# meyer-lab/cmtf-pls

Hardware: AMD Instinct MI355X
Metric: nipals_iters_per_sec (higher is better)
Workload: dtype f32

## Files before the change

cmtf_pls_amd/_lib.py:

```python
from __future__ import annotations

import ctypes
import os
from ctypes import c_char_p, c_double, c_int, c_int64, c_size_t, c_uint32, c_uint64, c_void_p

_HERE = os.path.dirname(os.path.abspath(__file__))
LIB_PATH = os.environ.get("CMTFPLS_LIB") or os.path.join(_HERE, "lib", "libcmtfpls.so")

_P = c_void_p

class XcovBlock(ctypes.Structure):
    _fields_ = [("S", _P), ("S2", _P), ("colcnt", _P), ("n_samples", c_double), ("order", c_int), ("A", c_int), ("B", c_int),
                ("n_squarings", c_int), ("Z", _P), ("wA", _P), ("wB", _P), ("info", _P)]


class KfoldState(ctypes.Structure):
    _fields_ = [("I", c_int), ("A", c_int), ("B", c_int), ("M", c_int), ("K", c_int), ("R", c_int)] + [
        (name, _P) for name in ("fold_of", "S", "mean", "Yk", "Gy", "WA", "WB", "Q", "Wa", "Wb", "T", "Gt", "coef", "Rm", "tm",
                                "Tout", "vec", "n_iter", "status", "part")]


class CvCoupledBlock(ctypes.Structure):
    _fields_ = [("X", _P), ("order", c_int), ("A", c_int), ("B", c_int)]

# ... 42 lines not shown
    "cmtfpls_project_rows2_idx_f64": (c_int, [_P, c_int, c_int, _P, _P, _P, _P, c_int, c_int, _P, _P, _P, _P, c_int64, c_int, _P, c_int, _P]),
    "cmtfpls_allreduce_sum_f64": (c_int, [_P, _P, c_size_t, _P]),
    "cmtfpls_allreduce_sum_f32": (c_int, [_P, _P, c_size_t, _P]),
    "cmtfpls_axpy_scalar_f64": (c_int, [_P, c_int64, _P, _P, _P]),
    "cmtfpls_xcov_deflate_f32": (c_int, [_P, c_int64, c_int, c_int, _P, c_int, c_int, _P, _P, _P, _P, _P, _P, c_size_t, _P]),
    "cmtfpls_xcov_deflate_f64": (c_int, [_P, c_int64, c_int, c_int, _P, c_int, c_int, _P, _P, _P, _P, _P, _P, c_size_t, _P]),
    "cmtfpls_xcov_stats_workspace_bytes": (c_size_t, [c_int64, c_int64, c_int]),
    "cmtfpls_xcov_stats_f32": (c_int, [_P, c_int64, c_int64, _P, c_int, c_int, _P, _P, _P, c_size_t, _P]),
    "cmtfpls_xcov_stats_f64": (c_int, [_P, c_int64, c_int64, _P, c_int, c_int, _P, _P, _P, c_size_t, _P]),
    "cmtfpls_xcov_ssq_workspace_bytes": (c_size_t, [c_int64, c_int64, c_int]),
    "cmtfpls_xcov_ssq_f32": (c_int, [_P, c_int64, c_int64, _P, c_int, c_int, _P, _P, _P, _P, c_size_t, _P]),
    "cmtfpls_xcov_ssq_f64": (c_int, [_P, c_int64, c_int64, _P, c_int, c_int, _P, _P, _P, _P, c_size_t, _P]),
    "cmtfpls_score_contract_workspace_bytes": (c_size_t, [c_int64, c_int64]),
    "cmtfpls_score_contract_f32": (c_int, [_P, c_int64, c_int, c_int, _P, _P, _P, _P, _P, c_double, _P, _P, _P, _P, c_size_t, _P]),
    "cmtfpls_score_contract_f64": (c_int, [_P, c_int64, c_int, c_int, _P, _P, _P, _P, _P, c_double, _P, _P, _P, _P, c_size_t, _P]),
    "cmtfpls_kr_axpy_f64": (c_int, [_P, c_int, c_int, _P, _P, c_int, c_int, _P, _P]),
    "cmtfpls_xcov_f32_mixed": (c_int, [_P, c_int64, c_int64, _P, c_int, c_int, _P, c_int, _P, c_size_t, _P]),
    "cmtfpls_mttkrp_f32_mixed": (c_int, [_P, c_int64, c_int, c_int, _P, _P, c_int, _P, c_int, _P]),
    "cmtfpls_mttkrp_f32": (c_int, [_P, c_int64, c_int, c_int, _P, _P, c_int, _P, c_int, _P]),
    "cmtfpls_mttkrp_f64": (c_int, [_P, c_int64, c_int, c_int, _P, _P, c_int, _P, c_int, _P]),
    "cmtfpls_score_f32": (c_int, [_P, c_int64, c_int, c_int, _P, _P, _P, _P, _P]),
    "cmtfpls_score_f64": (c_int, [_P, c_int64, c_int, c_int, _P, _P, _P, _P, _P]),
    "cmtfpls_score_s_f64": (c_int, [_P, c_int, c_int, c_int, _P, _P, _P, _P]),
    "cmtfpls_deflate_contract_workspace_bytes": (c_size_t, [c_int64, c_int64]),
    "cmtfpls_deflate_contract_yq_f32": (c_int, [_P, c_int64, c_int, c_int, _P, _P, _P, _P, c_int, c_int, _P, _P, c_int, _P, _P, c_size_t, _P]),
    "cmtfpls_deflate_contract_yq_f64": (c_int, [_P, c_int64, c_int, c_int, _P, _P, _P, _P, c_int, c_int, _P, _P, c_int, _P, _P, c_size_t, _P]),
    "cmtfpls_score_gram_f32": (c_int, [_P, c_int64, c_int, c_int, _P, _P, _P, _P, _P, c_int, c_int, _P, _P]),
    "cmtfpls_score_gram_f64": (c_int, [_P, c_int64, c_int, c_int, _P, _P, _P, _P, _P, c_int, c_int, _P, _P]),
    "cmtfpls_q_update_f64": (c_int, [_P, c_int, c_int, _P, c_int, _P, _P, _P, _P]),
    "cmtfpls_deflate_f32": (c_int, [_P, c_int64, c_int, c_int, _P, _P, _P, _P, _P]),
# ... 128 lines not shown
```

cmtf_pls_amd/backend.py:

```python
from __future__ import annotations

import ctypes
from typing import Optional, Tuple

import torch

from . import _lib

_SUFFIX = {torch.float32: "f32", torch.float64: "f64"}


def _ptr(t: Optional[torch.Tensor]):
    return None if t is None else t.data_ptr()


def _int_pairs(pairs):
    flat = [int(v) for p in pairs for v in p]
    return (ctypes.c_int * len(flat))(*flat)


class HipBackend:
    name = "hip"

    def __init__(self, device: Optional[torch.device] = None):
# ... 297 lines not shown
        if rc == 4:
            return None
        _lib.check(rc, "mttkrp")
        return out

    def score(self, X2, A, B, wA, wB, rowcnt, out) -> torch.Tensor:
        _lib.check(self._fn("score", X2)(_ptr(X2), X2.shape[0], A, B, _ptr(wA), _ptr(wB), _ptr(rowcnt), _ptr(out), self._stream()), "score")
        return out

    def score_s(self, S, A, B, wA, wB, out) -> torch.Tensor:
        assert S.dtype == torch.float64 and S.is_contiguous()
        _lib.check(self.lib.cmtfpls_score_s_f64(_ptr(S), S.shape[0], A, B, _ptr(wA), _ptr(wB), _ptr(out), self._stream()), "score_s")
        return out

    def score_contract(self, X2, A, B, wA, wB, shift, t, Z, sub_own=None, add_other=None, alpha: float = 1.0,
                       csum: Optional[torch.Tensor] = None) -> Optional[torch.Tensor]:
        I, P = X2.shape
        if not X2.is_contiguous() or P != A * B:
            return None
        for v in (sub_own, add_other):
            assert v is None or (v.is_contiguous() and v.numel() == I and v.dtype == torch.float64)
        nbytes = self.lib.cmtfpls_score_contract_workspace_bytes(I, P)
        ws = self._workspace("score_contract", max(nbytes, 256))
        rc = self._fn("score_contract", X2)(_ptr(X2), I, A, B, _ptr(wA), _ptr(wB), _ptr(shift), _ptr(sub_own), _ptr(add_other), float(alpha),
                                            _ptr(t), _ptr(Z), _ptr(csum), _ptr(ws), ws.numel(), self._stream())
        if rc == 4:
            return None
        _lib.check(rc, "score_contract")
        return Z

    def score_gram(self, X2, A, B, wA, wB, rowcnt, out, Y: torch.Tensor, qpart: torch.Tensor) -> Optional[torch.Tensor]:
        assert qpart.numel() >= self.n_partials * Y.shape[1] and qpart.is_contiguous()
        rc = self._fn("score_gram", X2)(_ptr(X2), X2.shape[0], A, B, _ptr(wA), _ptr(wB), _ptr(rowcnt), _ptr(out),
                                        _ptr(Y), Y.stride(0), Y.shape[1], _ptr(qpart), self._stream())
        if rc == 4:
            return None
        _lib.check(rc, "score_gram")
        return out

    def q_update(self, q: torch.Tensor, qpart: Optional[torch.Tensor] = None, normalize: bool = True,
                 G: Optional[torch.Tensor] = None, q_prev: Optional[torch.Tensor] = None,
                 du2: Optional[torch.Tensor] = None, nparts: Optional[int] = None) -> None:
        M = q.numel()
# ... 619 lines not shown
```

cmtf_pls_amd/csrc/scorecontract.hip:

```cpp
#include "common.hpp"

namespace cmtfpls {

void launch_reduce_rows(const double* part, int nrows, int64_t P, double* out, hipStream_t st);

constexpr int kScGrid = 256;

template <int CTRL>
__device__ __forceinline__ double dpp_move(double v) {
  const uint64_t b = __double_as_longlong(v);
  const uint32_t lo = (uint32_t)__builtin_amdgcn_update_dpp(0, (int)(uint32_t)b, CTRL, 0xf, 0xf, false);
  const uint32_t hi = (uint32_t)__builtin_amdgcn_update_dpp(0, (int)(uint32_t)(b >> 32), CTRL, 0xf, 0xf, false);
  return __longlong_as_double(((uint64_t)hi << 32) | lo);
}
__device__ __forceinline__ double row16_sum(double v) {
  v += dpp_move<0xB1>(v);
  v += dpp_move<0x4E>(v);
  v += dpp_move<0x141>(v);
  v += dpp_move<0x140>(v);
  return v;
}

constexpr int kScLdsA = 2048;
template <typename T, int NV, bool KC, bool WL = false>
__global__ __launch_bounds__(1024) void score_contract_rows_kernel(const T* __restrict__ X, int64_t I, unsigned P, int B,
                                                                  const double* __restrict__ wA, const double* __restrict__ wB,
                                                                  const double* __restrict__ shift, const double* __restrict__ sub_own,
                                                                  const double* __restrict__ add_other, double alpha,
                                                                  double* __restrict__ t, double* __restrict__ part,
                                                                  double* __restrict__ csum_part) {
  __shared__ double red[2][16];
  __shared__ double wls[WL ? kScLdsA : 1];
  constexpr int V = VecOf<T>::N;
  using VT = Pack<T, V>;
  constexpr unsigned stride = 1024u * V;
  const unsigned c0 = threadIdx.x * V;
  const int lane = threadIdx.x & 63, wv = threadIdx.x >> 6;
  double wa[WL ? 1 : NV], wb[KC ? 1 : NV][V], acc[NV][V];
  bool ok[NV];
  const unsigned j0 = c0 / (unsigned)B, jstep = stride / (unsigned)B;
  if constexpr (WL) {
    for (unsigned j = threadIdx.x; j < NV * jstep; j += 1024) wls[(j % jstep) * NV + j / jstep] = wA[j];
    __syncthreads();
  }
#pragma unroll
// ... 7 lines not shown
      if (!KC || n == 0) wb[KC ? 0 : n][e] = wB[cg % (unsigned)B + e];
      acc[n][e] = 0.0;
    }
  }
  const double sh = shift ? shift[0] : 0.0;
  unsigned col[WL ? 1 : NV];
  if constexpr (!WL) {
#pragma unroll
    for (int n = 0; n < NV; ++n) col[n] = ok[n] ? c0 + n * stride : 0u;
  }
  const int64_t step = gridDim.x;
  int64_t r = blockIdx.x;
  VT bufA[NV], bufB[NV];
  int parity = 0;
  double csum = 0.0;
  auto load = [&](VT (&buf)[NV], int64_t row) {
#pragma unroll
    for (int n = 0; n < NV; ++n) {
      if constexpr (WL) {
        const uint64_t o = (uint64_t)(row * (int64_t)P + (int64_t)n * stride);
        const uint64_t ou = ((uint64_t)__builtin_amdgcn_readfirstlane((uint32_t)(o >> 32)) << 32) | __builtin_amdgcn_readfirstlane((uint32_t)o);
        buf[n] = ld_stream(reinterpret_cast<const VT*>(X + ou + c0));
      } else {
        buf[n] = ld_stream(reinterpret_cast<const VT*>(X + row * (int64_t)P + col[n]));
      }
    }
  };
  auto use = [&](VT (&buf)[NV], int64_t row) {
    double d = 0.0;
#pragma unroll
    for (int n = 0; n < NV; ++n) {
      double dn = 0.0;
#pragma unroll
      for (int e = 0; e < V; ++e) dn = fma((double)buf[n].e[e], wb[KC ? 0 : n][e], dn);
      d = fma(WL ? wls[j0 * NV + n] : wa[WL ? 0 : n], dn, d);
    }
    d = wave_sum(d);
    if (lane == 0) red[parity][wv] = d;
    __syncthreads();
    double ti = row16_sum(red[parity][lane & 15]) - sh;
    parity ^= 1;
    if (sub_own) ti -= sub_own[row];
    if (threadIdx.x == 0) t[row] = ti;
    if (add_other) ti += add_other[row];
    ti *= alpha;
    csum += ti;
    if constexpr (sizeof(T) == 4) {
#pragma unroll
      for (int n = 0; n < NV; ++n)
#pragma unroll
        for (int e = 0; e < V; ++e) asm volatile("" : "+v"(buf[n].e[e]));
    }
#pragma unroll
    for (int n = 0; n < NV; ++n)
#pragma unroll
      for (int e = 0; e < V; ++e) acc[n][e] = fma(ti, (double)buf[n].e[e], acc[n][e]);
  };
  const int64_t last = I - 1;
  if (r < I) load(bufA, r);
  while (r < I) {
    const int64_t r1 = r + step;
    load(bufB, r1 < I ? r1 : last);
    use(bufA, r);
    if (r1 >= I) break;
    const int64_t r2 = r1 + step;
    load(bufA, r2 < I ? r2 : last);
    use(bufB, r1);
    r = r2;
  }
  if (csum_part && threadIdx.x == 0) csum_part[blockIdx.x] = csum;
  double* __restrict__ prow = part + (int64_t)blockIdx.x * P + c0;
#pragma unroll
  for (int n = 0; n < NV; ++n)
    if (ok[n]) {
#pragma unroll
      for (int e = 0; e < V; ++e) prow[n * stride + e] = acc[n][e];
    }
}

constexpr unsigned long long kXchEmpty = ~0ull;
constexpr int kSplitMaxG = 16;
constexpr int kSplitSpinLimit = 1 << 21;

__global__ __launch_bounds__(256) void xch_preset_kernel(unsigned long long* __restrict__ p, int64_t n) {
  for (int64_t i = (int64_t)blockIdx.x * 256 + threadIdx.x; i < n; i += (int64_t)gridDim.x * 256) p[i] = kXchEmpty;
// ... 125 lines not shown
}

static int split_cus() {
  static int cus = 0;
  if (cus == 0) {
    int dev = 0, n = 0;
    if (hipGetDevice(&dev) != hipSuccess || hipDeviceGetAttribute(&n, hipDeviceAttributeMultiprocessorCount, dev) != hipSuccess || n <= 0) n = 256;
    cus = n;
  }
  return cus;
}

template <typename T>
static int run_score_contract(const T* X, int64_t I, int A, int B, const double* wA, const double* wB, const double* shift,
                              const double* sub_own, const double* add_other, double alpha, double* t, double* Z, double* csum,
                              void* ws, size_t ws_bytes, hipStream_t st) {
  if (!X || !wA || !wB || !t || !Z || I <= 0 || A <= 0 || B <= 0) { set_error("score_contract: bad argument"); return CMTFPLS_EINVAL; }
  constexpr int V = 16 / (int)sizeof(T);
  const int64_t P = (int64_t)A * B;
  const int64_t stride = (int64_t)1024 * V;
  const int nv = (int)((P + stride - 1) / stride);
  constexpr int kMaxNV = (V == 4) ? 4 : 8;
  if ((B % V) != 0 || P < stride / 2 || P >= ((int64_t)1 << 31) || (reinterpret_cast<uintptr_t>(X) & 15) != 0) {
    set_error("score_contract: shape outside the row-in-registers form; use score + mode0_contract");
    return CMTFPLS_EUNSUPPORTED;
  }
  const bool kc = (stride % B) == 0;
  if (nv > kMaxNV) {
    const int NVS = (sizeof(T) == 4 && !kc) ? 2 : 4;
    const int G = (nv + NVS - 1) / NVS;
    const int cus = split_cus() < kScGrid ? split_cus() : kScGrid;
    const int S = (int)(I < cus / G ? I : cus / G);
    if (G > kSplitMaxG || S < 1) {
      set_error("score_contract: row beyond 16 workgroups' registers; use score + mode0_contract");
      return CMTFPLS_EUNSUPPORTED;
    }
    const size_t need = ((size_t)S * (P + 1) + (size_t)I * G) * sizeof(double);
    if (!ws || ws_bytes < need) { set_error("score_contract: workspace too small"); return CMTFPLS_EWORKSPACE; }
    double* part = static_cast<double*>(ws);
    double* csum_part = part + (size_t)S * P;
    unsigned long long* xch = reinterpret_cast<unsigned long long*>(csum_part + S);
    hipLaunchKernelGGL(xch_preset_kernel, dim3((unsigned)(((int64_t)I * G + 2047) / 2048)), dim3(256), 0, st, xch, (int64_t)I * G);
// ... 1 lines not shown
  hipLaunchKernelGGL((score_contract_split_kernel<T, NVV, KCC, LG>), dim3(S * G), dim3(1024), 0, st, X, I, (unsigned)P, B, G, wA, wB, \
                     shift, sub_own, add_other, alpha, t, part, csum ? csum_part : nullptr, xch)
    if constexpr (sizeof(T) == 8) {
      if (kc) SPL(4, true, 2);
      else SPL(4, false, 1);
    } else {
      if (kc) SPL(4, true, 1);
      else SPL(2, false, 2);
    }
#undef SPL
    launch_reduce_rows(part, S, P, Z, st);
    if (csum) launch_reduce_rows(csum_part, S, 1, csum, st);
    return check_launch("score_contract (split rows)");
  }
  const int grid = (int)(I < kScGrid ? I : kScGrid);
  if (!ws || ws_bytes < (size_t)grid * (P + 1) * sizeof(double)) { set_error("score_contract: workspace too small"); return CMTFPLS_EWORKSPACE; }
  double* part = static_cast<double*>(ws);
  double* csum_part = csum ? part + (size_t)grid * P : nullptr;
#define SCL(NVV)                                                                                                                  \
  do {                                                                                                                            \
    if (kc) hipLaunchKernelGGL((score_contract_rows_kernel<T, NVV, true>), dim3(grid), dim3(1024), 0, st, X, I, (unsigned)P, B, wA, wB, shift, sub_own, add_other, alpha, t, part, csum_part); \
    else hipLaunchKernelGGL((score_contract_rows_kernel<T, NVV, false>), dim3(grid), dim3(1024), 0, st, X, I, (unsigned)P, B, wA, wB, shift, sub_own, add_other, alpha, t, part, csum_part); \
  } while (0)
  if (nv <= 1) SCL(1);
  else if (nv <= 2) SCL(2);
  else if (nv <= 4) SCL(4);
  else if constexpr (kMaxNV >= 8) {
    if (kc && P == 8 * stride && A <= kScLdsA)
      hipLaunchKernelGGL((score_contract_rows_kernel<T, 8, true, true>), dim3(grid), dim3(1024), 0, st, X, I, (unsigned)P, B, wA, wB, shift, sub_own, add_other, alpha, t, part, csum_part);
    else SCL(8);
  }
#undef SCL
  launch_reduce_rows(part, grid, P, Z, st);
  if (csum) launch_reduce_rows(csum_part, grid, 1, csum, st);
  return check_launch("score_contract");
}

}

using namespace cmtfpls;

extern "C" {
size_t cmtfpls_score_contract_workspace_bytes(int64_t I, int64_t P) {
  if (I <= 0 || P <= 0) return 0;
  return ((size_t)(I < kScGrid ? I : kScGrid) * (size_t)(P + 1) + (size_t)I * kSplitMaxG) * sizeof(double);
}
int cmtfpls_score_contract_f32(const float* X, int64_t I, int A, int B, const double* wA, const double* wB, const double* shift,
                               const double* sub_own, const double* add_other, double alpha, double* t, double* Z, double* csum,
                               void* ws, size_t ws_bytes, void* stream) {
  return run_score_contract<float>(X, I, A, B, wA, wB, shift, sub_own, add_other, alpha, t, Z, csum, ws, ws_bytes, (hipStream_t)stream);
}
int cmtfpls_score_contract_f64(const double* X, int64_t I, int A, int B, const double* wA, const double* wB, const double* shift,
                               const double* sub_own, const double* add_other, double alpha, double* t, double* Z, double* csum,
                               void* ws, size_t ws_bytes, void* stream) {
  return run_score_contract<double>(X, I, A, B, wA, wB, shift, sub_own, add_other, alpha, t, Z, csum, ws, ws_bytes, (hipStream_t)stream);
}
}
```

cmtf_pls_amd/csrc/small.hip:

```cpp
#include "common.hpp"

namespace cmtfpls {

void launch_reduce_rows(const double* part, int nrows, int64_t P, double* out, hipStream_t st);

constexpr int kSmallBlocks = 128;
constexpr int kMaxGramDim = 64;
constexpr size_t kSmallWsBytes = (size_t)kSmallBlocks * kMaxGramDim * kMaxGramDim * sizeof(double);

__global__ __launch_bounds__(256) void gram_tn_kernel(const double* __restrict__ A, int lda, int a,
                                                     const double* __restrict__ B, int ldb, int b,
                                                     int64_t I, double* __restrict__ part, int TR) {
  extern __shared__ double lds[];
  double* As = lds;
  double* Bs = lds + TR * a;
  const int ab = a * b;
  const int64_t rows_per = (I + gridDim.x - 1) / gridDim.x;
  const int64_t r0 = (int64_t)blockIdx.x * rows_per;
  const int64_t r1 = (r0 + rows_per < I) ? r0 + rows_per : I;
  double acc[16];
#pragma unroll
  for (int s = 0; s < 16; ++s) acc[s] = 0.0;
  for (int64_t rb = r0; rb < r1; rb += TR) {
    const int nr = (int)((r1 - rb < TR) ? r1 - rb : TR);
// ... 207 lines not shown
    if (lane < M) {
      q[lane] = v;
      if (G) dq[lane] = v - q_prev[lane];
    }
  }
  if (G) {
    __syncthreads();
    double sacc = 0.0;
    for (int idx = tid; idx < M * M; idx += 1024) {
      const int i = idx / M, j = idx - i * M;
      sacc = fma(dq[i] * G[idx], dq[j], sacc);
    }
    sacc = block_sum(sacc, red);
    if (tid == 0) du2[0] = sacc;
  }
}

__global__ __launch_bounds__(256) void s_downdate_kernel(double* __restrict__ S, int M, int64_t P, int B,
                                                        const double* __restrict__ ya, const double* __restrict__ wA,
                                                        const double* __restrict__ wB, const double* __restrict__ q,
                                                        const double* __restrict__ v) {
  const int64_t c = (int64_t)blockIdx.x * 256 + threadIdx.x;
  if (c >= P) return;
  const double w = wA[c / B] * wB[c % B];
  const double vc = v[c];
  for (int m = 0; m < M; ++m) {
    double sv = S[(int64_t)m * P + c];
    sv = fma(-ya[m], w, sv);
    sv = fma(-q[m], vc, sv);
    S[(int64_t)m * P + c] = sv;
// ... 224 lines not shown
```

cmtf_pls_amd/fitrun.py:

```python
from __future__ import annotations

import math
from typing import Dict, List, Optional

import numpy as np
import torch

from .fitrun_xcov import XcovMixin
from .state import BlockState, FitState, split_trailing, validate_limits


class FitRun(XcovMixin):

    def __init__(self, eng: NipalsEngine, Xs: List[torch.Tensor], Y: torch.Tensor, n_components: int, coupled: bool,
                 algorithm: str = "direct", owned: Optional[List[bool]] = None, allow_raw: bool = True):
        be, comm = eng.be, eng.comm
        Xs = list(Xs)
        owned = [True] * len(Xs) if owned is None else list(owned)
        if algorithm not in ("direct", "xcov"):
            raise ValueError("algorithm must be 'direct' or 'xcov'")
        self.algorithm_requested = self.algorithm = algorithm
        self.notes: List[str] = []
        validate_limits([tuple(X.shape) for X in Xs], n_components)
        self.eng, self.Xs, self.Y, self.R, self.coupled = eng, Xs, Y, n_components, coupled
# ... 136 lines not shown
                self.one.fill_(1.0)
                self.vs = [be.empty(blk.A * blk.B) for blk in self.blocks]
                self._nowrite = eng.opt.xcov_nowrite and hasattr(be, "kr_axpy") and R <= 64
                if self._nowrite:
                    self.dot_log = be.zeros(R, 1 + len(self.blocks))
                    self.Gw = be.empty(R * R)
                    self._G_last = None
                    self._one_read = R > 1 and eng.opt.xcov_one_read and hasattr(be, "score_contract")
                    if self._one_read:
                        self._fused_b = max(range(len(self.blocks)), key=lambda b: self.blocks[b].A * self.blocks[b].B)
                        P0 = self.blocks[self._fused_b].A * self.blocks[self._fused_b].B
                        self.ps = be.empty(P0)
                        self.Rm = be.zeros(P0, R)
                        self.corr = be.empty(I)
                        self.csum = be.empty(1)
            assert self._nowrite or not self.raw, "an uncentred X needs the form of the loop that never writes it"

    def _blocks_from_one_read(self, Xs: List[torch.Tensor]) -> Optional[List[BlockState]]:
        be, comm = self.eng.be, self.eng.comm
        blocks, n = [], float(self.n_total)
        for b, X in enumerate(Xs):
            I = X.shape[0]
            X2 = X.view(I, -1)
            P = X2.shape[1]
            out = be.xcov_stats(X2, self.Y, out=be.empty(self.M, P))
            if out is None:
                return None
            S, stats = out
            comm.allreduce(stats)
            colsum, colsq = stats[:P], stats[P:]
            ssq = (colsq - colsum * colsum / n).sum().reshape(1)
# ... 483 lines not shown
            rep["x_passes_per_component"] = ("1 read + write (deflation fused with the next contraction)" if self._fused
                                             else "1 read + write (deflation)")
            rep["x_copy"] = "centred private copy"
        else:
            nowrite = bool(getattr(self, "_nowrite", False))
            one_read = nowrite and bool(getattr(self, "_one_read", False))
            any_miss = any(b.has_miss for b in self.blocks)
            rep["x_copy"] = "none: the caller's uncentred tensor is read in place" if self.raw else "centred private copy"
            rep["raw"] = bool(self.raw)
            rep["x_written"] = not nowrite
            rep["s_carried"] = bool(self._s_carry)
            rep["s_build"] = ("per component (missing values)" if any_miss else "first component only") + \
                             (f", {(self.M + 63) // 64} response tiles of <= 64" if self.M > 64 else "") + \
                             (", [Y, Y * rowscale] in one pass" if any(x is not None for x in self.S12) else "")
            rep["one_read"] = one_read
            rep["stats_with_s"] = bool(getattr(self, "_stats_with_s", False))
            if nowrite:
                rep["x_passes_per_component"] = ("1 read (largest block); 2 reads (other blocks)" if one_read and nb > 1 else
                                                 "1 read" if one_read else "2 reads")
            elif any_miss and nb == 1 and getattr(self, "_deflate_build_ok", True) and self.S12[0] is not None and eng.opt.xcov_deflate_build:
                rep["x_passes_per_component"] = "1 read + 1 read + write (deflation inside the rebuild of S)"
            elif any_miss:
                rep["x_passes_per_component"] = "1 read + write (score + deflation) + S rebuild reads"
            else:
                rep["x_passes_per_component"] = "1 read + 1 read + write"
            rep["pipelined"] = bool(getattr(self, "_pipelined", False))
            if rep["pipelined"]:
                rep["pipeline"] = dict(self.pipeline_stats)
            if not rep["pipelined"] and eng.opt.xcov_pipeline:
                why = ("graph replay requested" if self.use_graphs else "more than 64 responses" if self.M > 64 else
# ... 14 lines not shown
```

cmtf_pls_amd/fitrun_xcov.py:

```python
from __future__ import annotations

import math
from typing import Optional

import torch


class XcovMixin:
    def _iterate_xcov(self, it: int) -> Optional[float]:
        be = self.eng.be
        self._executed += 1

        blk0 = self.blocks[0]
        composite = (len(self.blocks) == 1 and len(blk0.shape) == 3 and not blk0.has_miss and self.M <= 64
                     and self.qn.data_ptr() == self.Tq.data_ptr() and hasattr(be, "xcov_iterate"))

        par = self._parity
        q_cur, q_new = self.qx[par], self.qx[par ^ 1]

        def seg(first: bool):
            if composite:
                be.xcov_iterate(self.S[0], blk0.A, blk0.B, q_cur, self.Zs[0], self.wA[0], self.wB[0], self.status[1:3],
                                self.sq_budget[0], q_new, self.Gy, self.status[0:1], first)
                return
# ... 184 lines not shown
                    comm.allreduce(self.vs[b])
                    be.s_downdate(self.S[b], blk.A, blk.B, ya_g, self.wA[b], self.wB[b], self.q, self.vs[b])
            self._s_ready = carried
        else:
            for b, blk in enumerate(self.blocks):
                ssqs.append(be.deflate(self.X2[b], blk.A, blk.B, self.t, self.wA[b], self.wB[b]))
        self._log_ssq(a, ssqs, ssqy)

    def _finish_xcov_nowrite(self, a: int) -> None:
        be, comm = self.eng.be, self.eng.comm
        self.q = self.qc
        I, R, k = self.I, self.R, a + 1
        nb = len(self.blocks)
        self._store_loadings(a)
        fused_b = self._fused_b if (getattr(self, "_one_read", False) and k < R) else -1
        one_read = False
        for b in [x for x in range(nb) if x != fused_b] + ([fused_b] if fused_b >= 0 else []):
            blk = self.blocks[b]
            mw = None
            if self.raw:
                mw = be.score_s(blk.mean.view(1, -1), blk.A, blk.B, self.wA[b], self.wB[b], be.empty(1))
            g = None
            if a > 0 and hasattr(be, "kr_gram_row"):
                for m, L in enumerate(blk.loadings):
                    be.kr_gram_row(L, a, self.Gw, first=(m == 0))
                g = self.Gw[:a]
            elif a > 0:
                for m, L in enumerate(blk.loadings):
                    be.kr_gram(L, self.Gw, first=(m == 0))
                g = self.Gw.view(R, R)[a, :a]
            if b == fused_b:
                corr = others = None
                if a > 0:
                    be.rowdot(self.T[:, :a], g, self.corr, None)
                    corr = self.corr
                if nb == 2:
                    others = self.Ts[1 - b]
                elif nb > 2:
                    others = self.Ts[[x for x in range(nb) if x != b]].sum(dim=0)
                one_read = be.score_contract(self.X2[b], blk.A, blk.B, self.wA[b], self.wB[b], mw, self.Ts[b], self.ps,
                                             sub_own=corr, add_other=others, alpha=1.0 / nb,
                                             csum=self.csum if self.raw else None) is not None
                if one_read:
                    continue
                self._one_read = False
            be.score(self.X2[b], blk.A, blk.B, self.wA[b], self.wB[b], None, self.Ts[b])
            if mw is not None:
                be.axpy_scalar(self.Ts[b], mw)
            if a > 0:
                be.y_deflate(self.Ts[b].view(I, 1), self.T, a, g, self.one)
        single = self.t.data_ptr() == self.Ts.data_ptr()
        if not single:
            be.scores_mean(self.Ts, self.t)
        if one_read:
            comm.allreduce(self.ps)
            if self.raw:
                be.axpy_scalar(self.ps, comm.allreduce(self.csum), self.blocks[fused_b].mean)
            self.Rm[:, a].copy_(self.ps)
        be.rowdot(self.Y, self.q, self.u, None)
        be.gram_tn(self.t, self.t, out=self.dot_log[a, 0:1])
        for b in range(nb):
            if single:
                self.dot_log[a, 1 + b].copy_(self.dot_log[a, 0])
            else:
                be.gram_tn(self.Ts[b], self.t, out=self.dot_log[a, 1 + b: 2 + b])
        self.T[:, a].copy_(self.t)
        self.U[:, a].copy_(self.u)
        self.Q[:, a].copy_(self.q)
        Ta = self.T[:, :k]
        ya = be.gram_tn(self.Y, self.t).reshape(-1)
        b_dev, ya_g = self._inner_regression(a, extra=ya)
        if k < R and not (one_read and nb == 1):
            be.rowdot(Ta, b_dev, self.yhat.view(-1), None)
        ssqy = be.y_deflate(self.Y, self.T, k, b_dev, self.q)
        if k < R:
            c = be.gram_tn(self._G_last, b_dev).reshape(-1)
            for b, blk in enumerate(self.blocks):
                WA, WB = self.eng._kr_operands(blk, R)
                if one_read and b == fused_b:
                    be.rowdot(self.Rm[:, :k], b_dev, self.vs[b], None)
                else:
                    be.mode0_contract(self.X2[b], self.yhat.view(-1), False, out=self.vs[b])
                    comm.allreduce(self.vs[b])
                    if self.raw:
                        be.axpy_scalar(self.vs[b], comm.allreduce(be.total(self.yhat.view(-1))), blk.mean)
                be.kr_axpy(self.vs[b], blk.A, blk.B, WA, WB, k, c)
# ... 4 lines not shown
```

cmtf_pls_amd/options.py:

```python
from __future__ import annotations

from dataclasses import dataclass, replace
from typing import Optional


@dataclass(frozen=True)
class EngineOptions:
    small_fit: bool = True
    small_fit_elements: int = 1 << 15
    xcov_nowrite: bool = True
    xcov_raw: bool = True
    xcov_raw_max_offset: float = 1e4
    project_raw_max_offset: float = 1e4
    xcov_one_read: bool = True
    xcov_pair_build: bool = True
    xcov_ssq_with_s: bool = True
    xcov_stats_with_s: bool = True
    xcov_deflate_build: bool = True
    xcov_pipeline: bool = True
    capture_collectives: bool = False
    project_split_rows: bool = True
    masked_folds: bool = False
    masked_folds_coupled: bool = False
    coupled_permutations: bool = False
    tensor_folds: bool = False
    tensor_folds_coupled: bool = False

    def but(self, **changes) -> "EngineOptions":
        return replace(self, **changes)
# ... 14 lines not shown
```

include/cmtfpls.h:

```cpp
#ifndef CMTFPLS_H
#define CMTFPLS_H

#include <stddef.h>
#include <stdint.h>

#ifdef __cplusplus
extern "C" {
#endif

#define CMTFPLS_OK 0
#define CMTFPLS_EINVAL 1
#define CMTFPLS_EWORKSPACE 2
#define CMTFPLS_EHIP 3
#define CMTFPLS_EUNSUPPORTED 4

int cmtfpls_abi_version(void);
const char* cmtfpls_last_error(void);
int cmtfpls_clear_error(void);
int cmtfpls_status_to_host(const void* src, void* dst_host, size_t bytes, void* event, void* stream);

size_t cmtfpls_colstats_workspace_bytes(int64_t I, int64_t P);
int cmtfpls_colstats_f32(const float* X, int64_t I, int64_t P, double* colsum, double* colcnt,
                         void* ws, size_t ws_bytes, void* stream);
int cmtfpls_colstats_f64(const double* X, int64_t I, int64_t P, double* colsum, double* colcnt,
// ... 68 lines not shown
  double* info;
} cmtfpls_xcov_block;
int cmtfpls_xcov_iterate_blocks_f64(const cmtfpls_xcov_block* blocks, int nb, int M, const double* q_cur, double* tq, double* q_new,
                                    const double* G, double* du2, int first, void* ws_rank1, size_t ws_rank1_bytes, void* stream);
int cmtfpls_s_downdate_f64(double* S, int M, int A, int B, const double* ya, const double* wA, const double* wB,
                           const double* q, const double* v, void* stream);
int cmtfpls_kr_axpy_f64(double* v, int A, int B, const double* WA, const double* WB, int ld, int k, const double* coef, void* stream);
int cmtfpls_axpy_scalar_f64(double* y, int64_t n, const double* a, const double* x, void* stream);
size_t cmtfpls_score_contract_workspace_bytes(int64_t I, int64_t P);
int cmtfpls_score_contract_f32(const float* X, int64_t I, int A, int B, const double* wA, const double* wB, const double* shift,
                               const double* sub_own, const double* add_other, double alpha, double* t, double* Z, double* csum,
                               void* ws, size_t ws_bytes, void* stream);
int cmtfpls_score_contract_f64(const double* X, int64_t I, int A, int B, const double* wA, const double* wB, const double* shift,
                               const double* sub_own, const double* add_other, double alpha, double* t, double* Z, double* csum,
                               void* ws, size_t ws_bytes, void* stream);
int cmtfpls_xcov_f32_mixed(const float* X, int64_t I, int64_t P, const double* Y, int ldy, int M, double* S,
                           int masked, void* ws, size_t ws_bytes, void* stream);
int cmtfpls_mttkrp_f32_mixed(const float* X, int64_t I, int A, int B, const double* WA, const double* WB, int R,
                             double* out, int ldo, void* stream);

int cmtfpls_mttkrp_f32(const float* X, int64_t I, int A, int B, const double* WA, const double* WB, int R,
                       double* out, int ldo, void* stream);
int cmtfpls_mttkrp_f64(const double* X, int64_t I, int A, int B, const double* WA, const double* WB, int R,
                       double* out, int ldo, void* stream);

int cmtfpls_score_f32(const float* X, int64_t I, int A, int B, const double* wA, const double* wB,
                      const double* rowcnt, double* t, void* stream);
int cmtfpls_score_f64(const double* X, int64_t I, int A, int B, const double* wA, const double* wB,
                      const double* rowcnt, double* t, void* stream);
int cmtfpls_score_s_f64(const double* S, int M, int A, int B, const double* wA, const double* wB, double* tq, void* stream);
// ... 239 lines not shown
```

Before: 765.6.

## Fuse per-component score epilogue into the score-contract X pass

Adds an epilogue variant of the score-contract kernel that, while streaming X rows, also computes u = Y q, writes the T and U columns, and accumulates t·t, Yᵀt and Tᵀt partials using spare wavefronts. A single-block reduce kernel then produces dots, ya and the inner-regression Gram. This replaces several separate small launches (rowdot, gram_tn, copies, inner regression) per component and is meant to cut launch overhead and extra reads of Y and T. In exchange the row-loop kernel does more work and loads per row, and the path applies only to single, uncoupled, unsharded order-3 fits.

```diff
diff --git a/cmtf_pls_amd/_lib.py b/cmtf_pls_amd/_lib.py
--- a/cmtf_pls_amd/_lib.py
+++ b/cmtf_pls_amd/_lib.py
@@ -80,6 +80,10 @@
     "cmtfpls_score_contract_workspace_bytes": (c_size_t, [c_int64, c_int64]),
     "cmtfpls_score_contract_f32": (c_int, [_P, c_int64, c_int, c_int, _P, _P, _P, _P, _P, c_double, _P, _P, _P, _P, c_size_t, _P]),
     "cmtfpls_score_contract_f64": (c_int, [_P, c_int64, c_int, c_int, _P, _P, _P, _P, _P, c_double, _P, _P, _P, _P, c_size_t, _P]),
+    "cmtfpls_score_contract_epilogue_plan": (c_int, [c_int, c_int64, c_int, c_int, c_int, c_int, ctypes.POINTER(c_int), ctypes.POINTER(c_int),
+                                                     ctypes.POINTER(c_size_t), c_char_p, c_size_t]),
+    "cmtfpls_score_contract_epilogue_f32": (c_int, [_P, c_int64, c_int, c_int, _P, _P, _P, _P, _P, _P, _P, _P, c_int, c_int, _P, _P, _P, c_int, _P, c_int, c_int, _P, c_int, _P, _P, c_int, _P, _P, c_size_t, _P]),
+    "cmtfpls_score_contract_epilogue_f64": (c_int, [_P, c_int64, c_int, c_int, _P, _P, _P, _P, _P, _P, _P, _P, c_int, c_int, _P, _P, _P, c_int, _P, c_int, c_int, _P, c_int, _P, _P, c_int, _P, _P, c_size_t, _P]),
     "cmtfpls_kr_axpy_f64": (c_int, [_P, c_int, c_int, _P, _P, c_int, c_int, _P, _P]),
     "cmtfpls_xcov_f32_mixed": (c_int, [_P, c_int64, c_int64, _P, c_int, c_int, _P, c_int, _P, c_size_t, _P]),
     "cmtfpls_mttkrp_f32_mixed": (c_int, [_P, c_int64, c_int, c_int, _P, _P, c_int, _P, c_int, _P]),
diff --git a/cmtf_pls_amd/backend.py b/cmtf_pls_amd/backend.py
--- a/cmtf_pls_amd/backend.py
+++ b/cmtf_pls_amd/backend.py
@@ -335,12 +335,15 @@
         return out
 
     def score_contract(self, X2, A, B, wA, wB, shift, t, Z, sub_own=None, add_other=None, alpha: float = 1.0,
-                       csum: Optional[torch.Tensor] = None) -> Optional[torch.Tensor]:
+                       csum: Optional[torch.Tensor] = None, epilogue: Optional[dict] = None) -> Optional[torch.Tensor]:
         I, P = X2.shape
         if not X2.is_contiguous() or P != A * B:
             return None
         for v in (sub_own, add_other):
             assert v is None or (v.is_contiguous() and v.numel() == I and v.dtype == torch.float64)
+        if epilogue is not None:
+            assert add_other is None and alpha == 1.0
+            return self._score_contract_epilogue(X2, A, B, wA, wB, shift, t, Z, sub_own, csum, **epilogue)
         nbytes = self.lib.cmtfpls_score_contract_workspace_bytes(I, P)
         ws = self._workspace("score_contract", max(nbytes, 256))
         rc = self._fn("score_contract", X2)(_ptr(X2), I, A, B, _ptr(wA), _ptr(wB), _ptr(shift), _ptr(sub_own), _ptr(add_other), float(alpha),
@@ -348,6 +351,32 @@
         if rc == 4:
             return None
         _lib.check(rc, "score_contract")
+        return Z
+
+    def score_contract_epilogue_plan(self, dtype, I: int, A: int, B: int, M: int, a: int) -> Optional[str]:
+        why = ctypes.create_string_buffer(128)
+        rc = self.lib.cmtfpls_score_contract_epilogue_plan(4 if dtype == torch.float32 else 8, int(I), int(A), int(B), int(M), int(a),
+                                                           None, None, None, why, len(why))
+        return None if rc == 0 else why.value.decode()
+
+    def _score_contract_epilogue(self, X2, A, B, wA, wB, shift, t, Z, sub_own, csum, Y, q, u, T, U, a: int, dots, ya, G, Gk
+                                 ) -> Optional[torch.Tensor]:
+        I, P = X2.shape
+        assert Y.stride(1) == 1 and T.stride(1) == 1 and U.stride(1) == 1 and G.stride(1) == 1 and Y.shape[0] == I == T.shape[0] == U.shape[0]
+        assert u.is_contiguous() and u.numel() == I and dots.is_contiguous() and ya.is_contiguous() and ya.numel() == Y.shape[1]
+        assert Gk.is_contiguous() and Gk.numel() >= (a + 1) * (a + 1) and q.is_contiguous() and q.numel() == Y.shape[1]
+        M = Y.shape[1]
+        nbytes = ctypes.c_size_t(0)
+        if self.lib.cmtfpls_score_contract_epilogue_plan(X2.element_size(), I, A, B, M, int(a), None, None, ctypes.byref(nbytes), None, 0) != 0:
+            return None
+        ws = self._workspace("score_contract", max(int(nbytes.value), 256))
+        rc = self._fn("score_contract_epilogue", X2)(_ptr(X2), I, A, B, _ptr(wA), _ptr(wB), _ptr(shift), _ptr(sub_own), _ptr(t), _ptr(Z),
+                                                     _ptr(csum), _ptr(Y), Y.stride(0), M, _ptr(q), _ptr(u), _ptr(T), T.stride(0), _ptr(U),
+                                                     U.stride(0), int(a), _ptr(dots), dots.numel(), _ptr(ya), _ptr(G), G.stride(0), _ptr(Gk),
+                                                     _ptr(ws), ws.numel(), self._stream())
+        if rc == 4:
+            return None
+        _lib.check(rc, "score_contract_epilogue")
         return Z
 
     def score_gram(self, X2, A, B, wA, wB, rowcnt, out, Y: torch.Tensor, qpart: torch.Tensor) -> Optional[torch.Tensor]:
diff --git a/cmtf_pls_amd/csrc/scorecontract.hip b/cmtf_pls_amd/csrc/scorecontract.hip
--- a/cmtf_pls_amd/csrc/scorecontract.hip
+++ b/cmtf_pls_amd/csrc/scorecontract.hip
@@ -1,10 +1,21 @@
 #include "common.hpp"
+#include "scorecontract_plan.hpp"
 
 namespace cmtfpls {
 
 void launch_reduce_rows(const double* part, int nrows, int64_t P, double* out, hipStream_t st);
-
-constexpr int kScGrid = 256;
+void launch_xcov_epilogue_reduce(const double* part, int nblk, int M, int a, double* dots, int ndots, double* ya, double* G, int ldg,
+                                 double* Gk, hipStream_t st);
+
+struct ScEpi {
+  const double* Y;
+  const double* q;
+  double* Tm;
+  double* u;
+  double* U;
+  double* part;
+  int ldy, M, ldt, ldu, a;
+};
 
 template <int CTRL>
 __device__ __forceinline__ double dpp_move(double v) {
@@ -22,13 +33,13 @@
 }
 
 constexpr int kScLdsA = 2048;
-template <typename T, int NV, bool KC, bool WL = false>
+template <typename T, int NV, bool KC, bool WL = false, bool EPI = false>
 __global__ __launch_bounds__(1024) void score_contract_rows_kernel(const T* __restrict__ X, int64_t I, unsigned P, int B,
                                                                   const double* __restrict__ wA, const double* __restrict__ wB,
                                                                   const double* __restrict__ shift, const double* __restrict__ sub_own,
                                                                   const double* __restrict__ add_other, double alpha,
                                                                   double* __restrict__ t, double* __restrict__ part,
-                                                                  double* __restrict__ csum_part) {
+                                                                  double* __restrict__ csum_part, ScEpi ep) {
   __shared__ double red[2][16];
   __shared__ double wls[WL ? kScLdsA : 1];
   constexpr int V = VecOf<T>::N;
@@ -66,7 +77,19 @@
   VT bufA[NV], bufB[NV];
   int parity = 0;
   double csum = 0.0;
-  auto load = [&](VT (&buf)[NV], int64_t row) {
+  const double* eptr = nullptr;
+  int eld = 0;
+  double evA = 0.0, evB = 0.0, eacc = 0.0;
+  if constexpr (EPI) {
+    const bool ont = wv == 3 && ep.a > 0;
+    const int hi = ont ? ep.a - 1 : ep.M - 1;
+    const int el = (wv >= 1 && wv <= 3) ? (lane < hi ? lane : hi) : 0;
+    eptr = (ont ? (const double*)ep.Tm : ep.Y) + el;
+    eld = ont ? ep.ldt : ep.ldy;
+    if (wv == 1) eacc = ep.q[lane < ep.M ? lane : ep.M - 1];
+  }
+  auto load = [&](VT (&buf)[NV], double& ev, int64_t row) {
+    if constexpr (EPI) ev = eptr[row * (int64_t)eld];
 #pragma unroll
     for (int n = 0; n < NV; ++n) {
       if constexpr (WL) {
@@ -78,7 +101,7 @@
       }
     }
   };
-  auto use = [&](VT (&buf)[NV], int64_t row) {
+  auto use = [&](VT (&buf)[NV], double ev, int64_t row) {
     double d = 0.0;
 #pragma unroll
     for (int n = 0; n < NV; ++n) {
@@ -94,6 +117,26 @@
     parity ^= 1;
     if (sub_own) ti -= sub_own[row];
     if (threadIdx.x == 0) t[row] = ti;
+    if constexpr (EPI) {
+      if (threadIdx.x == 0) ep.Tm[row * ep.ldt + ep.a] = ti;
+      if (wv == 1) {
+        double s = 0.0;
+        const uint64_t yb = (uint64_t)__double_as_longlong(ev), qb = (uint64_t)__double_as_longlong(eacc);
+        for (int m = 0; m < ep.M; ++m) {
+          const uint64_t ym = ((uint64_t)(uint32_t)__builtin_amdgcn_readlane((int)(uint32_t)(yb >> 32), m) << 32) |
+                              (uint32_t)__builtin_amdgcn_readlane((int)(uint32_t)yb, m);
+          const uint64_t qm = ((uint64_t)(uint32_t)__builtin_amdgcn_readlane((int)(uint32_t)(qb >> 32), m) << 32) |
+                              (uint32_t)__builtin_amdgcn_readlane((int)(uint32_t)qb, m);
+          s = fma(__longlong_as_double((long long)ym), __longlong_as_double((long long)qm), s);
+        }
+        if (lane == 0) {
+          ep.u[row] = s;
+          ep.U[row * ep.ldu + ep.a] = s;
+        }
+      } else if (wv <= 3) {
+        eacc = fma(ti, wv == 0 ? ti : ev, eacc);
+      }
+    }
     if (add_other) ti += add_other[row];
     ti *= alpha;
     csum += ti;
@@ -109,18 +152,24 @@
       for (int e = 0; e < V; ++e) acc[n][e] = fma(ti, (double)buf[n].e[e], acc[n][e]);
   };
   const int64_t last = I - 1;
-  if (r < I) load(bufA, r);
+  if (r < I) load(bufA, evA, r);
   while (r < I) {
     const int64_t r1 = r + step;
-    load(bufB, r1 < I ? r1 : last);
-    use(bufA, r);
+    load(bufB, evB, r1 < I ? r1 : last);
+    use(bufA, evA, r);
     if (r1 >= I) break;
     const int64_t r2 = r1 + step;
-    load(bufA, r2 < I ? r2 : last);
-    use(bufB, r1);
+    load(bufA, evA, r2 < I ? r2 : last);
+    use(bufB, evB, r1);
     r = r2;
   }
   if (csum_part && threadIdx.x == 0) csum_part[blockIdx.x] = csum;
+  if constexpr (EPI) {
+    double* __restrict__ er = ep.part + (int64_t)blockIdx.x * (1 + ep.M + ep.a);
+    if (threadIdx.x == 0) er[0] = eacc;
+    if (wv == 2 && lane < ep.M) er[1 + lane] = eacc;
+    if (wv == 3 && lane < ep.a) er[1 + ep.M + lane] = eacc;
+  }
   double* __restrict__ prow = part + (int64_t)blockIdx.x * P + c0;
 #pragma unroll
   for (int n = 0; n < NV; ++n)
@@ -276,7 +325,7 @@
 template <typename T>
 static int run_score_contract(const T* X, int64_t I, int A, int B, const double* wA, const double* wB, const double* shift,
                               const double* sub_own, const double* add_other, double alpha, double* t, double* Z, double* csum,
-                              void* ws, size_t ws_bytes, hipStream_t st) {
+                              void* ws, size_t ws_bytes, hipStream_t st, ScEpi* epi = nullptr) {
   if (!X || !wA || !wB || !t || !Z || I <= 0 || A <= 0 || B <= 0) { set_error("score_contract: bad argument"); return CMTFPLS_EINVAL; }
   constexpr int V = 16 / (int)sizeof(T);
   const int64_t P = (int64_t)A * B;
@@ -288,6 +337,7 @@
     return CMTFPLS_EUNSUPPORTED;
   }
   const bool kc = (stride % B) == 0;
+  if (nv > kMaxNV && epi) { set_error("score_contract_epilogue: the X pass takes the split-row form"); return CMTFPLS_EUNSUPPORTED; }
   if (nv > kMaxNV) {
     const int NVS = (sizeof(T) == 4 && !kc) ? 2 : 4;
     const int G = (nv + NVS - 1) / NVS;
@@ -319,23 +369,35 @@
     return check_launch("score_contract (split rows)");
   }
   const int grid = (int)(I < kScGrid ? I : kScGrid);
-  if (!ws || ws_bytes < (size_t)grid * (P + 1) * sizeof(double)) { set_error("score_contract: workspace too small"); return CMTFPLS_EWORKSPACE; }
+  size_t need = (size_t)grid * (P + 1) * sizeof(double);
+  if (epi) need = plan_score_contract_epilogue((int)sizeof(T), I, A, B, epi->M, epi->a, true).ws_bytes;
+  if (!ws || ws_bytes < need) { set_error("score_contract: workspace too small"); return CMTFPLS_EWORKSPACE; }
   double* part = static_cast<double*>(ws);
   double* csum_part = csum ? part + (size_t)grid * P : nullptr;
+  ScEpi ep = {};
+  if (epi) {
+    epi->part = part + (size_t)grid * (P + 1);
+    ep = *epi;
+  }
+#define SCK(NVV, KCC, WLL)                                                                                                        \
+  do {                                                                                                                            \
+    if (epi) hipLaunchKernelGGL((score_contract_rows_kernel<T, NVV, KCC, WLL, true>), dim3(grid), dim3(1024), 0, st, X, I, (unsigned)P, B, wA, wB, shift, sub_own, add_other, alpha, t, part, csum_part, ep); \
+    else hipLaunchKernelGGL((score_contract_rows_kernel<T, NVV, KCC, WLL, false>), dim3(grid), dim3(1024), 0, st, X, I, (unsigned)P, B, wA, wB, shift, sub_own, add_other, alpha, t, part, csum_part, ep); \
+  } while (0)
 #define SCL(NVV)                                                                                                                  \
   do {                                                                                                                            \
-    if (kc) hipLaunchKernelGGL((score_contract_rows_kernel<T, NVV, true>), dim3(grid), dim3(1024), 0, st, X, I, (unsigned)P, B, wA, wB, shift, sub_own, add_other, alpha, t, part, csum_part); \
-    else hipLaunchKernelGGL((score_contract_rows_kernel<T, NVV, false>), dim3(grid), dim3(1024), 0, st, X, I, (unsigned)P, B, wA, wB, shift, sub_own, add_other, alpha, t, part, csum_part); \
+    if (kc) SCK(NVV, true, false);                                                                                                \
+    else SCK(NVV, false, false);                                                                                                  \
   } while (0)
   if (nv <= 1) SCL(1);
   else if (nv <= 2) SCL(2);
   else if (nv <= 4) SCL(4);
   else if constexpr (kMaxNV >= 8) {
-    if (kc && P == 8 * stride && A <= kScLdsA)
-      hipLaunchKernelGGL((score_contract_rows_kernel<T, 8, true, true>), dim3(grid), dim3(1024), 0, st, X, I, (unsigned)P, B, wA, wB, shift, sub_own, add_other, alpha, t, part, csum_part);
+    if (kc && P == 8 * stride && A <= kScLdsA) SCK(8, true, true);
     else SCL(8);
   }
 #undef SCL
+#undef SCK
   launch_reduce_rows(part, grid, P, Z, st);
   if (csum) launch_reduce_rows(csum_part, grid, 1, csum, st);
   return check_launch("score_contract");
@@ -360,4 +422,57 @@
                                void* ws, size_t ws_bytes, void* stream) {
   return run_score_contract<double>(X, I, A, B, wA, wB, shift, sub_own, add_other, alpha, t, Z, csum, ws, ws_bytes, (hipStream_t)stream);
 }
-}
+
+int cmtfpls_score_contract_epilogue_plan(int elem_size, int64_t I, int A, int B, int M, int a, int* grid, int* width, size_t* ws_bytes,
+                                         char* why, size_t why_len) {
+  const ScEpiPlan p = plan_score_contract_epilogue(elem_size, I, A, B, M, a, true);
+  if (grid) *grid = p.grid;
+  if (width) *width = p.width;
+  if (ws_bytes) *ws_bytes = p.ws_bytes;
+  if (why && why_len > 0) snprintf(why, why_len, "%s", p.why ? p.why : "");
+  return p.why ? CMTFPLS_EUNSUPPORTED : CMTFPLS_OK;
+}
+}
+
+namespace cmtfpls {
+template <typename T>
+static int run_score_contract_epilogue(const T* X, int64_t I, int A, int B, const double* wA, const double* wB, const double* shift,
+                                       const double* sub_own, double* t, double* Z, double* csum, const double* Y, int ldy, int M,
+                                       const double* q, double* u, double* Tm, int ldt, double* U, int ldu, int a, double* dots,
+                                       int ndots, double* ya, double* G, int ldg, double* Gk, void* ws, size_t ws_bytes, hipStream_t st) {
+  if (!X || !wA || !wB || !t || !Z || !Y || !q || !u || !Tm || !U || !dots || !ya || !G || !Gk || I <= 0 || A <= 0 || B <= 0 || M <= 0 ||
+      a < 0 || ldy < M || ldt <= a || ldu <= a || ldg <= a || ndots < 1) {
+    set_error("score_contract_epilogue: bad argument");
+    return CMTFPLS_EINVAL;
+  }
+  const ScEpiPlan p = plan_score_contract_epilogue((int)sizeof(T), I, A, B, M, a, (reinterpret_cast<uintptr_t>(X) & 15) == 0);
+  if (p.why) {
+    char msg[160];
+    snprintf(msg, sizeof(msg), "score_contract_epilogue: %s", p.why);
+    set_error(msg);
+    return CMTFPLS_EUNSUPPORTED;
+  }
+  ScEpi ep = {Y, q, Tm, u, U, nullptr, ldy, M, ldt, ldu, a};
+  const int rc = run_score_contract<T>(X, I, A, B, wA, wB, shift, sub_own, nullptr, 1.0, t, Z, csum, ws, ws_bytes, st, &ep);
+  if (rc != CMTFPLS_OK) return rc;
+  launch_xcov_epilogue_reduce(ep.part, p.grid, M, a, dots, ndots, ya, G, ldg, Gk, st);
+  return check_launch("score_contract_epilogue");
+}
+}
+
+extern "C" {
+int cmtfpls_score_contract_epilogue_f32(const float* X, int64_t I, int A, int B, const double* wA, const double* wB, const double* shift,
+                                        const double* sub_own, double* t, double* Z, double* csum, const double* Y, int ldy, int M,
+                                        const double* q, double* u, double* T, int ldt, double* U, int ldu, int a, double* dots, int ndots,
+                                        double* ya, double* G, int ldg, double* Gk, void* ws, size_t ws_bytes, void* stream) {
+  return run_score_contract_epilogue<float>(X, I, A, B, wA, wB, shift, sub_own, t, Z, csum, Y, ldy, M, q, u, T, ldt, U, ldu, a, dots, ndots,
+                                            ya, G, ldg, Gk, ws, ws_bytes, (hipStream_t)stream);
+}
+int cmtfpls_score_contract_epilogue_f64(const double* X, int64_t I, int A, int B, const double* wA, const double* wB, const double* shift,
+                                        const double* sub_own, double* t, double* Z, double* csum, const double* Y, int ldy, int M,
+                                        const double* q, double* u, double* T, int ldt, double* U, int ldu, int a, double* dots, int ndots,
+                                        double* ya, double* G, int ldg, double* Gk, void* ws, size_t ws_bytes, void* stream) {
+  return run_score_contract_epilogue<double>(X, I, A, B, wA, wB, shift, sub_own, t, Z, csum, Y, ldy, M, q, u, T, ldt, U, ldu, a, dots, ndots,
+                                             ya, G, ldg, Gk, ws, ws_bytes, (hipStream_t)stream);
+}
+}
diff --git a/cmtf_pls_amd/csrc/scorecontract_plan.hpp b/cmtf_pls_amd/csrc/scorecontract_plan.hpp
--- /dev/null
+++ b/cmtf_pls_amd/csrc/scorecontract_plan.hpp
@@ -0,0 +1,47 @@
+#pragma once
+#include <stddef.h>
+#include <stdint.h>
+
+namespace cmtfpls {
+
+constexpr int kScGrid = 256;
+constexpr int kScEpiMaxM = 64;
+constexpr int kScEpiMaxA = 64;
+
+struct ScEpiPlan {
+  const char* why;
+  int nv;
+  bool kc, wl;
+  int grid;
+  int width;
+  size_t csum_off, epi_off;
+  size_t ws_bytes;
+};
+
+inline ScEpiPlan plan_score_contract_epilogue(int elem, int64_t I, int A, int B, int M, int a, bool aligned16) {
+  ScEpiPlan p = {nullptr, 0, false, false, 0, 0, 0, 0, 0};
+  if ((elem != 4 && elem != 8) || I <= 0 || A <= 0 || B <= 0 || M <= 0 || a < 0) { p.why = "bad argument"; return p; }
+  if (M > kScEpiMaxM) { p.why = "more than 64 responses"; return p; }
+  if (a > kScEpiMaxA) { p.why = "more than 64 earlier components"; return p; }
+  const int V = 16 / elem;
+  const int64_t P = (int64_t)A * B;
+  const int64_t stride = (int64_t)1024 * V;
+  if ((B % V) != 0 || P < stride / 2 || P >= ((int64_t)1 << 31) || !aligned16) {
+    p.why = "row outside the rows-in-registers form of the X pass";
+    return p;
+  }
+  const int nv = (int)((P + stride - 1) / stride);
+  const int max_nv = (V == 4) ? 4 : 8;
+  if (nv > max_nv) { p.why = "the X pass takes the split-row form"; return p; }
+  p.kc = (stride % B) == 0;
+  p.nv = nv <= 1 ? 1 : nv <= 2 ? 2 : nv <= 4 ? 4 : 8;
+  p.wl = p.nv == 8 && p.kc && P == 8 * stride && A <= 2048;
+  p.grid = (int)(I < kScGrid ? I : kScGrid);
+  p.width = 1 + M + a;
+  p.csum_off = (size_t)p.grid * (size_t)P;
+  p.epi_off = p.csum_off + (size_t)p.grid;
+  p.ws_bytes = (p.epi_off + (size_t)p.grid * (size_t)p.width) * sizeof(double);
+  return p;
+}
+
+}
diff --git a/cmtf_pls_amd/csrc/small.hip b/cmtf_pls_amd/csrc/small.hip
--- a/cmtf_pls_amd/csrc/small.hip
+++ b/cmtf_pls_amd/csrc/small.hip
@@ -245,6 +245,39 @@
     sacc = block_sum(sacc, red);
     if (tid == 0) du2[0] = sacc;
   }
+}
+
+__global__ __launch_bounds__(256) void xcov_epilogue_reduce_kernel(const double* __restrict__ part, int nblk, int M, int a,
+                                                                  double* __restrict__ dots, int ndots, double* __restrict__ ya,
+                                                                  double* G, int ldg, double* __restrict__ Gk) {
+  __shared__ double row[1 + 64 + 64];
+  const int tid = threadIdx.x, W = 1 + M + a, k = a + 1;
+  if (tid < W) {
+    double s = 0.0;
+    const double* __restrict__ pc = part + tid;
+    for (int r = 0; r < nblk; r += 8) {
+      double v[8];
+#pragma unroll
+      for (int e = 0; e < 8; ++e) v[e] = pc[(int64_t)((r + e < nblk) ? r + e : nblk - 1) * W];
+#pragma unroll
+      for (int e = 0; e < 8; ++e) s += (r + e < nblk) ? v[e] : 0.0;
+    }
+    row[tid] = s;
+  }
+  __syncthreads();
+  if (tid < ndots) dots[tid] = row[0];
+  if (tid < M) ya[tid] = row[1 + tid];
+  for (int idx = tid; idx < k * k; idx += 256) {
+    const int i = idx / k, j = idx - i * k;
+    const double v = (i == a && j == a) ? row[0] : (i == a) ? row[1 + M + j] : (j == a) ? row[1 + M + i] : G[(int64_t)i * ldg + j];
+    Gk[idx] = v;
+    if (i == a || j == a) G[(int64_t)i * ldg + j] = v;
+  }
+}
+
+void launch_xcov_epilogue_reduce(const double* part, int nblk, int M, int a, double* dots, int ndots, double* ya, double* G, int ldg,
+                                 double* Gk, hipStream_t st) {
+  hipLaunchKernelGGL(xcov_epilogue_reduce_kernel, dim3(1), dim3(256), 0, st, part, nblk, M, a, dots, ndots, ya, G, ldg, Gk);
 }
 
 __global__ __launch_bounds__(256) void s_downdate_kernel(double* __restrict__ S, int M, int64_t P, int B,
diff --git a/cmtf_pls_amd/fitrun.py b/cmtf_pls_amd/fitrun.py
--- a/cmtf_pls_amd/fitrun.py
+++ b/cmtf_pls_amd/fitrun.py
@@ -174,7 +174,27 @@
                         self.Rm = be.zeros(P0, R)
                         self.corr = be.empty(I)
                         self.csum = be.empty(1)
+                        self._epi_why = self._epilogue_declined(P0)
+                        self._epi_taken = False
+                        if self._epi_why is None:
+                            self.ya = be.empty(M)
+                            self.Gt = be.zeros(R, R)
+                            self.Gk = be.empty(R * R)
             assert self._nowrite or not self.raw, "an uncentred X needs the form of the loop that never writes it"
+
+    def _epilogue_declined(self, P0: int) -> Optional[str]:
+        eng, be, blk = self.eng, self.eng.be, self.blocks[0]
+        if not eng.opt.xcov_epilogue:
+            return "switched off (EngineOptions.xcov_epilogue)"
+        if len(self.blocks) > 1 or self.coupled:
+            return "a coupled fit (the deflation uses the block-averaged score)"
+        if eng.comm.sharded:
+            return "a sharded fit (the sums are all-reduced)"
+        if len(blk.shape) != 3:
+            return "a block of order other than 3"
+        if not hasattr(be, "score_contract_epilogue_plan"):
+            return "a backend without the kernel"
+        return be.score_contract_epilogue_plan(blk.dtype, self.I, blk.A, blk.B, self.M, max(self.R - 2, 0))
 
     def _blocks_from_one_read(self, Xs: List[torch.Tensor]) -> Optional[List[BlockState]]:
         be, comm = self.eng.be, self.eng.comm
@@ -688,6 +708,9 @@
                              (f", {(self.M + 63) // 64} response tiles of <= 64" if self.M > 64 else "") + \
                              (", [Y, Y * rowscale] in one pass" if any(x is not None for x in self.S12) else "")
             rep["one_read"] = one_read
+            rep["epilogue"] = ("in the X pass" if getattr(self, "_epi_taken", False) else
+                               "separate launches: " + (getattr(self, "_epi_why", None) or
+                                                        ("blocks with missing values" if any_miss else "no one-read pass to carry it")))
             rep["stats_with_s"] = bool(getattr(self, "_stats_with_s", False))
             if nowrite:
                 rep["x_passes_per_component"] = ("1 read (largest block); 2 reads (other blocks)" if one_read and nb > 1 else
diff --git a/cmtf_pls_amd/fitrun_xcov.py b/cmtf_pls_amd/fitrun_xcov.py
--- a/cmtf_pls_amd/fitrun_xcov.py
+++ b/cmtf_pls_amd/fitrun_xcov.py
@@ -222,7 +222,7 @@
         nb = len(self.blocks)
         self._store_loadings(a)
         fused_b = self._fused_b if (getattr(self, "_one_read", False) and k < R) else -1
-        one_read = False
+        one_read = epi = False
         for b in [x for x in range(nb) if x != fused_b] + ([fused_b] if fused_b >= 0 else []):
             blk = self.blocks[b]
             mw = None
@@ -246,6 +246,15 @@
                     others = self.Ts[1 - b]
                 elif nb > 2:
                     others = self.Ts[[x for x in range(nb) if x != b]].sum(dim=0)
+                if self._epi_why is None:
+                    epi = be.score_contract(self.X2[b], blk.A, blk.B, self.wA[b], self.wB[b], mw, self.Ts[b], self.ps, sub_own=corr,
+                                            csum=self.csum if self.raw else None,
+                                            epilogue=dict(Y=self.Y, q=self.q, u=self.u, T=self.T, U=self.U, a=a, dots=self.dot_log[a],
+                                                          ya=self.ya, G=self.Gt, Gk=self.Gk)) is not None
+                    if epi:
+                        one_read = self._epi_taken = True
+                        continue
+                    self._epi_why = "the kernel declined the shape"
                 one_read = be.score_contract(self.X2[b], blk.A, blk.B, self.wA[b], self.wB[b], mw, self.Ts[b], self.ps,
                                              sub_own=corr, add_other=others, alpha=1.0 / nb,
                                              csum=self.csum if self.raw else None) is not None
@@ -265,19 +274,25 @@
             if self.raw:
                 be.axpy_scalar(self.ps, comm.allreduce(self.csum), self.blocks[fused_b].mean)
             self.Rm[:, a].copy_(self.ps)
-        be.rowdot(self.Y, self.q, self.u, None)
-        be.gram_tn(self.t, self.t, out=self.dot_log[a, 0:1])
-        for b in range(nb):
-            if single:
-                self.dot_log[a, 1 + b].copy_(self.dot_log[a, 0])
-            else:
-                be.gram_tn(self.Ts[b], self.t, out=self.dot_log[a, 1 + b: 2 + b])
-        self.T[:, a].copy_(self.t)
-        self.U[:, a].copy_(self.u)
         self.Q[:, a].copy_(self.q)
         Ta = self.T[:, :k]
-        ya = be.gram_tn(self.Y, self.t).reshape(-1)
-        b_dev, ya_g = self._inner_regression(a, extra=ya)
+        if epi:
+            ya_g, G = self.ya, self.Gk[: k * k].view(k, k)
+            b_dev = be.normal_solve(G, be.gram_tn(Ta, self.u).reshape(-1), out=self.b_dev[:k])
+            self.coef_dev[:k, a].copy_(b_dev)
+            self._G_last = G
+        else:
+            be.rowdot(self.Y, self.q, self.u, None)
+            be.gram_tn(self.t, self.t, out=self.dot_log[a, 0:1])
+            for b in range(nb):
+                if single:
+                    self.dot_log[a, 1 + b].copy_(self.dot_log[a, 0])
+                else:
+                    be.gram_tn(self.Ts[b], self.t, out=self.dot_log[a, 1 + b: 2 + b])
+            self.T[:, a].copy_(self.t)
+            self.U[:, a].copy_(self.u)
+            ya = be.gram_tn(self.Y, self.t).reshape(-1)
+            b_dev, ya_g = self._inner_regression(a, extra=ya)
         if k < R and not (one_read and nb == 1):
             be.rowdot(Ta, b_dev, self.yhat.view(-1), None)
         ssqy = be.y_deflate(self.Y, self.T, k, b_dev, self.q)
diff --git a/cmtf_pls_amd/options.py b/cmtf_pls_amd/options.py
--- a/cmtf_pls_amd/options.py
+++ b/cmtf_pls_amd/options.py
@@ -13,6 +13,7 @@
     xcov_raw_max_offset: float = 1e4
     project_raw_max_offset: float = 1e4
     xcov_one_read: bool = True
+    xcov_epilogue: bool = True
     xcov_pair_build: bool = True
     xcov_ssq_with_s: bool = True
     xcov_stats_with_s: bool = True
diff --git a/include/cmtfpls.h b/include/cmtfpls.h
--- a/include/cmtfpls.h
+++ b/include/cmtfpls.h
@@ -106,6 +106,16 @@
 int cmtfpls_score_contract_f64(const double* X, int64_t I, int A, int B, const double* wA, const double* wB, const double* shift,
                                const double* sub_own, const double* add_other, double alpha, double* t, double* Z, double* csum,
                                void* ws, size_t ws_bytes, void* stream);
+int cmtfpls_score_contract_epilogue_plan(int elem_size, int64_t I, int A, int B, int M, int a, int* grid, int* width, size_t* ws_bytes,
+                                         char* why, size_t why_len);
+int cmtfpls_score_contract_epilogue_f32(const float* X, int64_t I, int A, int B, const double* wA, const double* wB, const double* shift,
+                                        const double* sub_own, double* t, double* Z, double* csum, const double* Y, int ldy, int M,
+                                        const double* q, double* u, double* T, int ldt, double* U, int ldu, int a, double* dots, int ndots,
+                                        double* ya, double* G, int ldg, double* Gk, void* ws, size_t ws_bytes, void* stream);
+int cmtfpls_score_contract_epilogue_f64(const double* X, int64_t I, int A, int B, const double* wA, const double* wB, const double* shift,
+                                        const double* sub_own, double* t, double* Z, double* csum, const double* Y, int ldy, int M,
+                                        const double* q, double* u, double* T, int ldt, double* U, int ldu, int a, double* dots, int ndots,
+                                        double* ya, double* G, int ldg, double* Gk, void* ws, size_t ws_bytes, void* stream);
 int cmtfpls_xcov_f32_mixed(const float* X, int64_t I, int64_t P, const double* Y, int ldy, int M, double* S,
                            int masked, void* ws, size_t ws_bytes, void* stream);
 int cmtfpls_mttkrp_f32_mixed(const float* X, int64_t I, int A, int B, const double* WA, const double* WB, int R,
```

Result: no change. 765.8 (median of 2 runs) (+0.0%).
